# gsw4869/CUDA_LDPC

Measured on AMD Instinct MI355X. Metric: decoded codewords/sec (50-iter flooding min-sum, fixed iterations), higher is better.
Workload: dtype f32; 1 GPU; J4_L24_Z96 rate-0.833 batch=65536 codewords/GPU 50 iters Es/N0=3.0dB; kernel=qc_lds_halfrow-local<nf2,J4,L24,Z96,wc20,wv4,g4,w6>t768_lds79904, frames_per_gpu=65536

## Files before the change

__graft_entry__.py:

```python
import glob
import os
import subprocess
import sys

ROOT = os.path.dirname(os.path.abspath(__file__))
PKG = os.path.join(ROOT, "cuda_ldpc_amd")
CSRC = os.path.join(PKG, "csrc")
SO = os.path.join(PKG, "libcuda_ldpc_amd.so")
HIPCC = os.environ.get("HIPCC", "/opt/rocm/bin/hipcc")
HIP_FLAGS = ["-O3", "--offload-arch=gfx950", "-std=c++17", "-fPIC", "-shared", "-ffp-contract=off", "-Wall",
             "-Wno-unused-function"]


def _stale(target, sources):
    if not os.path.exists(target):
        return True
    t = os.path.getmtime(target)
    return any(os.path.getmtime(s) > t for s in sources)


def _unit_deps(unit):
    fam = os.path.basename(unit).split("_")[0]
    deps = [unit] + glob.glob(os.path.join(CSRC, "common*.hpp")) + glob.glob(os.path.join(ROOT, "include", "*.h"))
    with open(unit) as f:
        named = [line.split('"')[1] for line in f if line.startswith('#include "') and line.count('"') == 2]
    deps += [h for h in (os.path.join(CSRC, n) for n in named) if os.path.isfile(h)]
    for pat in ("*.hpp", "*.inc"):
        deps += [h for h in glob.glob(os.path.join(CSRC, pat)) if os.path.basename(h).startswith(fam + "_")]
    return deps


def build(force=False):
    units = sorted(glob.glob(os.path.join(CSRC, "*.hip")))
    objdir = os.path.join(ROOT, "build", "obj")
    os.makedirs(objdir, exist_ok=True)
    flags = [f for f in HIP_FLAGS if f != "-shared"]
    jobs, objs = [], []
    for u in units:
        o = os.path.join(objdir, os.path.basename(u)[:-4] + ".o")
        objs.append(o)
        if force or _stale(o, _unit_deps(u) + [os.path.abspath(__file__)]):
            cmd = [HIPCC] + flags + ["-I", os.path.join(ROOT, "include"), "-c", u, "-o", o]
            print("[build]", " ".join(cmd), flush=True)
            jobs.append((cmd, subprocess.Popen(cmd)))
    for cmd, p in jobs:
        if p.wait() != 0:
            raise subprocess.CalledProcessError(p.returncode, cmd)
    if force or jobs or _stale(SO, objs):
        cmd = [HIPCC, "--offload-arch=gfx950", "-shared", "-fPIC", "-o", SO] + objs
        print("[build]", " ".join(cmd), flush=True)
        subprocess.check_call(cmd)
    if ROOT not in sys.path:
        sys.path.insert(0, ROOT)
    from oracle import pyoracle
    pyoracle.build(force=force)
    import cuda_ldpc_amd
    return SO


def smoke():
    import numpy as np
    import torch
    if ROOT not in sys.path:
        sys.path.insert(0, ROOT)
    if not os.path.exists(SO):
        build()
    import cuda_ldpc_amd as C
    from oracle import pyoracle as orc
    assert torch.cuda.is_available(), "smoke() needs a GPU"
    torch.cuda.set_device(0)
    J, L, Z, F, iters = 4, 24, 96, 16, 10
    path = os.path.join(ROOT, "data", "bldpc", "J4_L24_Z96_BlockH.txt")
    seed = np.array([173, 173, 173], np.int32)
    y = orc.bldpc_awgn(seed, orc.bldpc_sigma(3.0), L * Z, F)
    want = orc.bldpc_decode(orc.BinaryCode(path, J, L, Z), y, F, iters, early_exit=0, want_app=True)
    code = C.BinaryCode.from_blockh(path, J, L, Z)
    yt = torch.from_numpy(y.reshape(L * Z, F)).cuda()
    for kern in (C.KERNEL_QC_LDS, C.KERNEL_TABLE):
        r = C.LDPC_Decoder_GPU(code, yt, max_iter=iters, exit_mode=C.EXIT_FIXED, kernel=kern, want_app=True)
        torch.cuda.synchronize()
        assert np.array_equal(r["D"].cpu().numpy().reshape(-1), want["D"]), "hard bits differ from the oracle"
        assert np.array_equal(r["app"].cpu().numpy().reshape(-1).view(np.uint32), want["app"].view(np.uint32)), "LLRs differ"
        print("[smoke] binary J4_L24_Z96 F=%d iters=%d kernel=%s: bit-exact vs oracle" % (F, iters, code.last_kernel))
    J, L, Z, F = 15, 30, 1280, 3
    path = os.path.join(ROOT, "data", "bldpc", "J15_L30_Z1280_BlockH.txt")
    seed = np.array([173, 173, 173], np.int32)
    y = orc.bldpc_awgn(seed, orc.bldpc_sigma(0.4), L * Z, F)
    want = orc.bldpc_decode(orc.BinaryCode(path, J, L, Z), y, F, 30, early_exit=1, want_app=True)
    code = C.BinaryCode.from_blockh(path, J, L, Z)
    r = C.LDPC_Decoder_GPU(code, torch.from_numpy(y.reshape(L * Z, F)).cuda(), max_iter=30, exit_mode=C.EXIT_BATCH_GLOBAL, want_app=True)
    torch.cuda.synchronize()
    assert r["iteraTime"] == want["it"] and np.array_equal(r["D"].cpu().numpy().reshape(-1), want["D"]), "J15_L30_Z1280 differs from the oracle"
    assert np.array_equal(r["app"].cpu().numpy().reshape(-1).view(np.uint32), want["app"].view(np.uint32)), "J15_L30_Z1280 LLRs differ"
    print("[smoke] binary J15_L30_Z1280 F=%d iteraTime=%d kernel=%s: bit-exact vs oracle" % (F, r["iteraTime"], code.last_kernel))
    from cuda_ldpc_amd import nbldpc as nb
    nbd = os.path.join(ROOT, "data", "nb")
    mul, _, _ = nb.GFInitial(64, os.path.join(nbd, "GF", "Arith.Table.GF.64.txt"))
    ncode = nb.NBCode(os.path.join(nbd, "BDS.576.288.GF.64.txt"), mul)
    ocode = orc.NBCode(os.path.join(nbd, "BDS.576.288.GF.64.txt"), os.path.join(nbd, "GF", "Arith.Table.GF.64.txt"))
    cw = np.loadtxt(os.path.join(nbd, "codeword_bds_gf64.txt"), dtype=np.int32)
    seed = np.array([173, 173, 173], np.int32)
    sigma = nb.sigma_of(3.0, ncode.rate)
    rx = np.stack([nb.AWGNChannel_CPU(seed, sigma, ncode, cw) for _ in range(4)])
    Lch = nb.Demodulate(ncode, torch.from_numpy(rx).cuda(), sigma)
    r = nb.Decoding_EMS(ncode, Lch, 2, 2, 20, want_state=True)
    torch.cuda.synchronize()
    for b in range(4):
        want = orc.nb_ems_decode(ocode, orc.nb_demodulate(ocode, rx[b], sigma), 2, 2, 20, want_state=True)
        assert np.array_equal(r["DecodeOutput"][b].cpu().numpy(), want["out"]), "NB symbols differ from the oracle"
        assert int(r["iter_number"][b]) == want["it"] and int(r["ok"][b]) == want["ok"]
        assert np.array_equal(r["LLR"][b].cpu().numpy().view(np.uint32), want["LLR"].view(np.uint32)), "NB LLRs differ"
    print("[smoke] NB BDS GF(64) N=96: 4 frames, iterations %s: bit-exact vs oracle" % r["iter_number"].cpu().tolist())
    r2 = nb.Decoding_EMS(ncode, Lch, 2, 2, 20, want_state="llr")
    torch.cuda.synchronize()
    for k in ("DecodeOutput", "iter_number", "ok"):
        assert torch.equal(r[k], r2[k]), "k_nb_ems2 differs from k_nb_ems: " + k
    assert torch.equal(r["LLR"].view(torch.int32), r2["LLR"].view(torch.int32)), "k_nb_ems2 LLRs differ"
    print("[smoke] NB BDS GF(64): two-frame pipeline kernel bit-exact as well")
    r4 = nb.Decoding_QSPA(ncode, Lch, 20, want_state=True)
    want = nb.Decoding_QSPA_host(ncode, Lch.cpu().numpy(), 20, want_state=True)
    torch.cuda.synchronize()
    for k in ("DecodeOutput", "iter_number", "ok"):
        assert np.array_equal(r4[k].cpu().numpy(), want[k]), "k_nb_qspa differs from the host statement: " + k
    for k in ("LLR", "L_c2v"):
        assert np.array_equal(r4[k].cpu().numpy().view(np.uint32), want[k].view(np.uint32)), "k_nb_qspa state differs: " + k
    print("[smoke] NB BDS GF(64): FHT sum-product, iterations %s: bit-exact vs host statement" % r4["iter_number"].cpu().tolist())
    r5 = nb.Decoding_QSPA(ncode, Lch, 20, want_state=True, layered=True)
    want = nb.Decoding_QSPA_host(ncode, Lch.cpu().numpy(), 20, want_state=True, layered=True)
    torch.cuda.synchronize()
    for k in ("DecodeOutput", "iter_number", "ok"):
        assert np.array_equal(r5[k].cpu().numpy(), want[k]), "k_nb_qspa_layered differs from the host statement: " + k
    for k in ("LLR", "L_c2v"):
        assert np.array_equal(r5[k].cpu().numpy().view(np.uint32), want[k].view(np.uint32)), "k_nb_qspa_layered state differs: " + k
    print("[smoke] NB BDS GF(64): layered FHT sum-product, iterations %s: bit-exact vs host statement" % r5["iter_number"].cpu().tolist())
    for layered, ref in ((False, r4), (True, r5)):
        rw = nb.Decoding_QSPA(ncode, Lch, 20, want_state=True, layered=layered, tier="workspace")
        torch.cuda.synchronize()
        assert ncode.last_kernel == ("k_nb_qspa_ws_layered" if layered else "k_nb_qspa_ws")
        for k in ("DecodeOutput", "iter_number", "ok", "LLR", "L_c2v"):
            assert torch.equal(rw[k].view(torch.int32), ref[k].view(torch.int32)), "%s differs from the LDS tier: %s" % (ncode.last_kernel, k)
    print("[smoke] NB BDS GF(64): FHT sum-product, workspace tier, both schedules: bit-exact vs the LDS tier")
    rm = C.RateMatch(ncode.N, [0, 5], range(88, 96))
    words = nb.PN_CodeWords(ncode, 1, 4, rate_match=rm)
    rxq = nb.AWGNChannel_RM_GPU(np.array([173, 173, 173], np.int32), 0.6, rm, 64, nb.RM_Select(rm, words))
    Lrm = nb.RM_Demodulate_Recover(rm, 64, rxq, 0.6)
    want = nb.RM_Demodulate_Recover_host(rm, 64, rxq.cpu().numpy(), 0.6)
    assert np.array_equal(Lrm.cpu().numpy().view(np.uint32), want.view(np.uint32)), "NB rate-matched L_ch differs from the host statement"
    r3 = nb.Decoding_EMS(ncode, Lrm, 2, 2, 20)
    torch.cuda.synchronize()
    assert int((r3["DecodeOutput"][:, [0, 5]] != 0).sum()) == 0, "a shortened symbol decoded to a non-zero element"
    print("[smoke] NB BDS GF(64) rate-matched (2 shortened, 8 punctured, E=%d): fused receive bit-exact vs host statement, %d of 4 frames ok"
          % (rm.E, int(r3["ok"].sum())))


if __name__ == "__main__":
    build(force="--force" in sys.argv)
    if "--smoke" in sys.argv:
        smoke()
```

cuda_ldpc_amd/csrc/bldpc_math.hpp:

```cpp
#pragma once
#include <hip/hip_runtime.h>
#include <stdint.h>
#define BLDPC_SELECT_FN __device__ __forceinline__
#include "bldpc_select.hpp"

namespace cldpc {

__device__ __forceinline__ uint32_t f2u(float x) { return __float_as_uint(x); }
__device__ __forceinline__ float u2f(uint32_t x) { return __uint_as_float(x); }

struct CnAcc {
    float m1, m2;
    uint32_t sgn;
    __device__ __forceinline__ void init()
    {
        m1 = __builtin_inff();
        m2 = __builtin_inff();
        sgn = 0u;
    }
    __device__ __forceinline__ void add(float q)
    {
        float a = __builtin_fabsf(q);
        sgn ^= f2u(q);
        m2 = __builtin_amdgcn_fmed3f(m1, m2, a);
        m1 = __builtin_fminf(m1, a);
    }
    __device__ __forceinline__ uint32_t key() const { return __builtin_amdgcn_bitop3_b32(f2u(m1), f2u(m2), sgn & 0x80000000u, 0x96); }
};

struct SelF32 {
    static __device__ __forceinline__ float min(float a, float b) { return __builtin_fminf(a, b); }
    static __device__ __forceinline__ float max(float a, float b) { return __builtin_fmaxf(a, b); }
    static __device__ __forceinline__ float min3(float a, float b, float c) { return __builtin_fminf(__builtin_fminf(a, b), c); }
    static __device__ __forceinline__ float med3(float a, float b, float c) { return __builtin_amdgcn_fmed3f(a, b, c); }
};

template <int N, int STRIDE> __device__ __forceinline__ void cn_two_smallest(const float *q, float &m1, float &m2, uint32_t &sgn)
{
    static_assert(N >= 2, "a check row half has at least two edges");
    float mag[N];
#pragma unroll
    for (int i = 0; i < N; i++) mag[i] = __builtin_fabsf(q[i * STRIDE]);
    two_smallest<SelF32, N, float>(mag, m1, m2);
#ifdef QC_XOR2
    sgn = 0u;
#pragma unroll
    for (int k = 0; k < N; k++) sgn ^= f2u(q[k * STRIDE]);
#else
    sgn = (N % 2) ? f2u(q[0]) : (f2u(q[0]) ^ f2u(q[STRIDE]));
#pragma unroll
    for (int k = 2 - (N % 2); k + 1 < N; k += 2) sgn = __builtin_amdgcn_bitop3_b32(sgn, f2u(q[k * STRIDE]), f2u(q[(k + 1) * STRIDE]), 0x96);
#endif
}

__device__ __forceinline__ float cn_out(float q, float m2, uint32_t key)
{
    return u2f(key ^ f2u(__builtin_amdgcn_fmed3f(q, -m2, m2)));
}

}
```

cuda_ldpc_amd/csrc/bldpc_qc2_body.inc:

```
template <typename GM, bool HIST, bool NORM = false> __global__ __launch_bounds__(GM::TPB, GM::MINW) void QC2_NAME(QcArgs a)
{
    constexpr int NF = GM::NF, L = GM::L, Z = GM::Z, WC = GM::WC, WV = GM::WV, GJ = GM::GJ, ZB = GM::ZB, WCH = GM::WCH;
    constexpr int RPT = GM::RPT, CPT = GM::CPT, NCG = GM::NCG, MSG = GM::MSG;
    static_assert(NF == 2, "the half-row kernel carries a frame pair per lane");
    constexpr bool LOC = GM::LOC;
    constexpr int NL = LOC ? CPT : 0;
    extern __shared__ __attribute__((aligned(16))) char lds[];
    const int chunk = (a.nWG + 7) >> 3;
#if QC2_PERSIST
    const int xcd = (int)(blockIdx.x & 7);
    int wg = 0;
#else
    const int wg = (int)(blockIdx.x & 7) * chunk + (int)(blockIdx.x >> 3);
    if (wg >= a.nWG) return;
#endif

    const int F = a.F;
    const int tid = threadIdx.x;
    const int wave = tid >> 6, lane = tid & 63, h = lane >> 5;
    const int jq = wave / ZB, t = (wave - jq * ZB) * 32 + (lane & 31);
    const int cg = jq * 2 + h;
#if QC2_PERSIST
    int f0 = 0;
#else
    const int f0 = wg * NF;
#endif
    int *lds_flag = reinterpret_cast<int *>(lds + GM::flag_byte);

    const int rbase = ((jq * WC + h * WCH) * Z + t) * MSG;
    const int sbase = (GM::Sslot + cg * Z + t) * MSG;
    int saddr[RPT][WCH];
    v2f32 Rr[RPT][WCH];
    int sst[LOC ? CPT : 1];
    int raddr[CPT][WV];
    {
        constexpr int NV = LOC ? CPT : 0, WVR = LOC ? WV - 1 : WV;
        int w[4 * GM::LW];
#pragma unroll
        for (int k = 0; k < GM::LW; k++) {
            const v4i32 x = a.lane[k * GM::TPB + tid];
            w[4 * k] = x.x; w[4 * k + 1] = x.y; w[4 * k + 2] = x.z; w[4 * k + 3] = x.w;
        }
#pragma unroll
        for (int cc = 0; cc < NV; cc++) sst[LOC ? cc : 0] = (GM::Sslot + w[cc]) * MSG;
#pragma unroll
        for (int rr = 0; rr < RPT; rr++)
#pragma unroll
            for (int i = 0; i < WCH; i++) saddr[rr][i] = w[NV + rr * WCH + i];
#pragma unroll
        for (int cc = 0; cc < CPT; cc++)
#pragma unroll
            for (int k = 0; k < WVR; k++) raddr[cc][k] = w[NV + RPT * WCH + cc * WVR + k];
    }
    v2f32 yreg[CPT];
    auto y_load = [&](int cc) -> v2f32 {
        const int n = LOC ? sst[LOC ? cc : 0] / MSG - GM::Sslot : (cg + cc * NCG) * Z + t;
        return a.y_raw ? *reinterpret_cast<const v2f32 *>(a.y_raw + (size_t)n * F + f0)
                       : *reinterpret_cast<const v2f32 *>(a.y + ((size_t)wg * (L * Z) + n) * NF);
    };
#if !QC2_PERSIST
#pragma unroll
    for (int cc = 0; cc < CPT; cc++) yreg[cc] = y_load(cc);
#endif
    if (tid < NF) {
        reinterpret_cast<float *>(lds)[GM::zero_slot * NF + tid] = 0.0f;
        reinterpret_cast<float *>(lds)[GM::inf_slot * NF + tid] = __builtin_inff();
        lds_flag[tid] = 0;
        lds_flag[NF + tid] = 0;
    }
    unsigned long long hist = 0;
    unsigned done = 0;
    constexpr unsigned ALL = (1u << NF) - 1u;
#ifdef QC_STAMPS
    int nst = 0;
    auto stamp = [&](unsigned long long v) { if (tid == 0 && nst < QC_STAMPS) a.stamps[(size_t)wg * QC_STAMPS + nst++] = v; };
    const unsigned hwid = __builtin_amdgcn_s_getreg((31 << 11) | 4), xcc = __builtin_amdgcn_s_getreg((31 << 11) | 20);
    stamp(((unsigned long long)xcc << 32) | hwid);
    stamp(__builtin_amdgcn_s_memtime());
    if (a.stagger && ((hwid >> 16) & 1))
        for (int i = 0; i < a.stagger; i += 64 * 16) __builtin_amdgcn_s_sleep(16);
#endif
#if !QC2_PERSIST
    __syncthreads();
#endif
#ifdef QC_STAMPS
    stamp(__builtin_amdgcn_s_memtime());
#endif

    auto vn_phase = [&](auto ZS, bool (&bad)[NF]) {
        constexpr bool zs = decltype(ZS)::value;
        constexpr int CB = (CPT * WV <= 12) ? CPT : 1;
        static_for<CPT / CB>([&](auto C0) {
            constexpr int c0 = decltype(C0)::value * CB;
            v2f32 R[CB][WV];
#pragma unroll
            for (int ci = 0; ci < CB; ci++)
#pragma unroll
                for (int k = 0; k < WV; k++) R[ci][k] = lds_ld2(raddr[c0 + ci][k]);
            static_for<CB>([&](auto CI) {
                constexpr int ci = decltype(CI)::value, cc = c0 + ci;
                v2f32 S = R[ci][0];
                if constexpr (zs) S = v2f32{0.0f, 0.0f} + S;
#pragma unroll
                for (int k = 1; k < WV; k++) S = S + R[ci][k];
                S = S + yreg[cc];
                lds_st2_imm<cc * NCG * Z * MSG>(sbase, S);
                if (HIST) {
                    const bool in_len = ((cg + cc * NCG) * Z + t) < a.length;
                    bad[0] = bad[0] || (in_len && S.x < 0);
                    bad[1] = bad[1] || (in_len && S.y < 0);
                }
            });
            if (CB < CPT) __builtin_amdgcn_sched_barrier(0);
        });
        asm volatile("s_waitcnt lgkmcnt(0)" ::: "memory");
    };
    v2f32 Sloc[LOC ? CPT : 1];
    const int jqs = __builtin_amdgcn_readfirstlane(jq);
    auto vn_phase_loc = [&](auto JJ, auto ZS, bool (&bad)[NF]) {
        constexpr int jj = decltype(JJ)::value;
        constexpr bool zs = decltype(ZS)::value;
        v2f32 R[CPT][WV - 1];
#pragma unroll
        for (int cc = 0; cc < CPT; cc++)
#pragma unroll
            for (int kk = 0; kk < WV - 1; kk++) R[cc][kk] = lds_ld2(raddr[cc][kk]);
        static_for<CPT>([&](auto CC) {
            constexpr int cc = decltype(CC)::value;
            v2f32 S = v2f32{0.0f, 0.0f};
            static_for<WV>([&](auto K) {
                constexpr int k = decltype(K)::value;
                v2f32 Rk;
                if constexpr (k == jj) Rk = Rr[0][cc];
                else Rk = R[cc][k - (k > jj ? 1 : 0)];
                if constexpr (k == 0 && !zs) S = Rk;
                else S = S + Rk;
            });
            S = S + yreg[cc];
            Sloc[LOC ? cc : 0] = S;
            lds_st2_imm<0>(sst[LOC ? cc : 0], S);
            if (HIST) {
                const bool in_len = (sst[LOC ? cc : 0] / MSG - GM::Sslot) < a.length;
                bad[0] = bad[0] || (in_len && S.x < 0);
                bad[1] = bad[1] || (in_len && S.y < 0);
            }
        });
        asm volatile("s_waitcnt lgkmcnt(0)" ::: "memory");
    };
    auto vn_first = [&](bool (&bad)[NF]) {
        static_for<CPT>([&](auto CC) {
            constexpr int cc = decltype(CC)::value;
            const v2f32 S = yreg[cc] + v2f32{0.0f, 0.0f};
            int n;
            if constexpr (LOC) {
                Sloc[LOC ? cc : 0] = S;
                lds_st2_imm<0>(sst[LOC ? cc : 0], S);
                n = sst[LOC ? cc : 0] / MSG - GM::Sslot;
            } else {
                lds_st2_imm<cc * NCG * Z * MSG>(sbase, S);
                n = (cg + cc * NCG) * Z + t;
            }
            if (HIST) {
                const bool in_len = n < a.length;
                bad[0] = bad[0] || (in_len && S.x < 0);
                bad[1] = bad[1] || (in_len && S.y < 0);
            }
        });
        asm volatile("s_waitcnt lgkmcnt(0)" ::: "memory");
    };
    auto vn_any = [&](bool (&bad)[NF]) {
        if constexpr (LOC) static_for<GM::J>([&](auto JJ) { if (jqs == decltype(JJ)::value) vn_phase_loc(JJ, std::true_type{}, bad); });
        else vn_phase(std::true_type{}, bad);
    };
    auto flags_publish = [&](const bool (&bad)[NF], int it) {
#pragma unroll
        for (int v = 0; v < NF; v++)
            if (bad[v]) lds_flag[(it & 1) * NF + v] = 1;
    };
    auto flags_collect = [&](int it) -> int {
        int flag = 0;
        if (tid < NF) {
            flag = lds_flag[(it & 1) * NF + tid] ? 0 : 1;
            lds_flag[((it + 1) & 1) * NF + tid] = 0;
            if (flag && it <= 64) hist |= (1ull << (it - 1));
        }
        return flag;
    };
    auto emit = [&](unsigned mask, bool (&bad)[NF]) {
        unsigned *obits = a.bits;
        float *oapp = a.app;
        asm volatile("" : "+s"(obits), "+s"(oapp));
#pragma unroll
        for (int cc = 0; cc < CPT; cc++) {
            const int n = (cg + cc * NCG) * Z + t;
            float S[NF];
            lds_ld<NF>(S, lds, sbase + cc * NCG * Z * MSG);
#pragma unroll
            for (int v = 0; v < NF; v++) {
                if (HIST && !((mask >> v) & 1u)) continue;
                const bool neg = S[v] < 0;
                if (!HIST) bad[v] = bad[v] || (n < a.length && neg);
                const unsigned long long m = __ballot(neg);
                if ((tid & 31) == 0 && f0 + v < F) obits[(size_t)(f0 + v) * GM::NW + (n >> 5)] = (unsigned)(m >> (tid & 32));
                if (oapp && f0 + v < F) oapp[(size_t)n * F + f0 + v] = S[v];
            }
        }
    };
    auto retire = [&](int it) -> bool {
        unsigned newly = 0;
#pragma unroll
        for (int v = 0; v < NF; v++)
            if (!lds_flag[(it & 1) * NF + v]) newly |= 1u << v;
        newly &= ~done;
        if (newly) {
            bool unused[NF];
            emit(newly, unused);
            if (tid < NF && ((newly >> tid) & 1u) && f0 + tid < F) a.iters[f0 + tid] = it;
            done |= newly;
        }
        return done == ALL;
    };

#if QC2_PERSIST
    for (;;) {
    if (tid == 0) lds_flag[0] = atomicAdd(&a.work[xcd], 1);
    __syncthreads();
    {
        const int ord = __builtin_amdgcn_readfirstlane(lds_flag[0]);
        if (ord >= chunk || xcd * chunk + ord >= a.nWG) break;
        wg = xcd * chunk + ord;
    }
    __syncthreads();
    f0 = wg * NF;
#pragma unroll
    for (int cc = 0; cc < CPT; cc++) yreg[cc] = y_load(cc);
    if (tid < NF) {
        lds_flag[tid] = 0;
        lds_flag[NF + tid] = 0;
    }
    hist = 0;
    done = 0;
    __syncthreads();
#endif
    auto iteration = [&](auto JJ, auto FIRST, int it) -> bool {
        constexpr bool first = decltype(FIRST)::value;
        bool bad[NF];
#pragma unroll
        for (int v = 0; v < NF; v++) bad[v] = false;
        __builtin_amdgcn_s_setprio(QC_PRIO_VN);
        if constexpr (first) vn_first(bad);
        else if constexpr (LOC) vn_phase_loc(JJ, std::bool_constant<HIST>{}, bad);
        else vn_phase(std::bool_constant<HIST>{}, bad);
        if (HIST) flags_publish(bad, it);
        __syncthreads();
        __builtin_amdgcn_s_setprio(QC_PRIO_CN);
#ifdef QC_STAMPS
        stamp(__builtin_amdgcn_s_memtime());
#endif
        if (HIST) {
            (void)flags_collect(it);
            if (a.per_frame && retire(it)) return true;
        }

#pragma unroll
        for (int rr = 0; rr < RPT; rr++) {
            CnAcc acc[NF];
            {
#ifdef QC2_CHK_SPLIT
                constexpr int CHK = (WCH > 6) ? (WCH + 1) / 2 : WCH;
#else
                constexpr int CHK = (WCH > 6 && !LOC) ? (WCH + 1) / 2 : WCH;
#endif
#pragma unroll
                for (int c0 = 0; c0 < WCH; c0 += CHK) {
                    v2f32 Sv[CHK];
#pragma unroll
                    for (int i = 0; i < CHK && c0 + i < WCH; i++) {
                        if (LOC && c0 + i < NL) Sv[i] = Sloc[LOC ? c0 + i : 0];
                        else Sv[i] = lds_ld2(saddr[rr][c0 + i]);
                    }
#pragma unroll
                    for (int i = 0; i < CHK && c0 + i < WCH; i++) Rr[rr][c0 + i] = first ? Sv[i] : Sv[i] - Rr[rr][c0 + i];
                    if (c0 + CHK < WCH) __builtin_amdgcn_sched_barrier(0);
                }
            }
#if QC_ACC_RUNNING
#pragma unroll
            for (int v = 0; v < NF; v++) acc[v].init();
#pragma unroll
            for (int i = 0; i < WCH; i++) {
                acc[0].add(Rr[rr][i].x);
                acc[1].add(Rr[rr][i].y);
            }
#else
            cn_two_smallest<WCH, 2>(reinterpret_cast<const float *>(&Rr[rr][0]), acc[0].m1, acc[0].m2, acc[0].sgn);
            cn_two_smallest<WCH, 2>(reinterpret_cast<const float *>(&Rr[rr][0]) + 1, acc[1].m1, acc[1].m2, acc[1].sgn);
#endif
            uint32_t a1 = f2u(acc[0].m1), b1 = f2u(acc[1].m1), a2 = f2u(acc[0].m2), b2 = f2u(acc[1].m2), as = acc[0].sgn, bs = acc[1].sgn;
            swap32(a1, b1);
            swap32(a2, b2);
            swap32(as, bs);
            const uint32_t m1 = min(a1, b1);
            uint32_t m2u = min(min(max(a1, b1), a2), b2);
            uint32_t keyu = __builtin_amdgcn_bitop3_b32(m1, m2u, __builtin_amdgcn_bitop3_b32(as, bs, 0x80000000u, 0x28), 0x96);
            uint32_t m2v = m2u, keyv = keyu;
            swap32(m2u, m2v);
            swap32(keyu, keyv);
            const float m2f[NF] = {u2f(m2u), u2f(m2v)};
            const uint32_t key[NF] = {keyu, keyv};
            __builtin_amdgcn_s_setprio(LOC ? QC_PRIO_WR_LOC : QC_PRIO_WR);
            static_for<RPT * WCH>([&](auto I) {
                constexpr int r_ = decltype(I)::value / WCH, i = decltype(I)::value % WCH;
                if (r_ != rr) return;
                v2f32 Rn;
                Rn.x = cn_out(Rr[rr][i].x, m2f[0], key[0]);
                Rn.y = cn_out(Rr[rr][i].y, m2f[1], key[1]);
                if constexpr (NORM) Rn = Rn * a.alpha;
                Rr[rr][i] = Rn;
                if constexpr (!(LOC && i < NL)) lds_st2_imm<(r_ * GJ * WC + i) * Z * MSG>(rbase, Rn);
            });
        }
        asm volatile("s_waitcnt lgkmcnt(0)" ::: "memory");
        __syncthreads();
#ifdef QC_STAMPS
        stamp(__builtin_amdgcn_s_memtime());
#endif
        return false;
    };
    const bool retired = a.max_iter > 1 && iteration(std::integral_constant<int, 0>{}, std::true_type{}, 1);
    auto iterate = [&](auto JJ) {
        for (int it = 2; it < a.max_iter; it++)
            if (iteration(JJ, std::false_type{}, it)) return;
    };
    if (!retired) {
        if constexpr (LOC) static_for<GM::J>([&](auto JJ) { if (jqs == decltype(JJ)::value) iterate(JJ); });
        else iterate(std::integral_constant<int, 0>{});
    }

    int flag = 0;
    if (!(HIST && done == ALL)) {
        bool bad[NF];
#pragma unroll
        for (int v = 0; v < NF; v++) bad[v] = false;
        if (a.max_iter > 1) vn_any(bad);
        else vn_first(bad);
        if (LOC) __syncthreads();
        emit(~done, bad);
        flags_publish(bad, a.max_iter);
        __syncthreads();
        flag = flags_collect(a.max_iter);
    }
#ifdef QC_STAMPS
    stamp(__builtin_amdgcn_s_memtime());
#endif
    if (tid < NF && f0 + tid < F) {
        const bool stopped = HIST && ((done >> tid) & 1u);
        a.D[(size_t)L * Z * F + f0 + tid] = stopped ? 1 : flag;
        if (HIST && a.hist) a.hist[f0 + tid] = hist;
        if (HIST && a.per_frame && !stopped) a.iters[f0 + tid] = a.max_iter;
    }
#if QC2_PERSIST
    __syncthreads();
    }
#endif
}
```

cuda_ldpc_amd/csrc/bldpc_select.hpp:

```cpp
#pragma once

#ifndef BLDPC_SELECT_FN
#define BLDPC_SELECT_FN inline
#endif

namespace cldpc {

template <typename P, int N, typename T> BLDPC_SELECT_FN void two_smallest(const T (&v)[N], T &m1, T &m2)
{
    static_assert(N >= 2, "two values at least");
    if constexpr (N == 2) {
        m1 = P::min(v[0], v[1]);
        m2 = P::max(v[0], v[1]);
    } else if constexpr (N == 3) {
        m1 = P::min3(v[0], v[1], v[2]);
        m2 = P::med3(v[0], v[1], v[2]);
    } else if constexpr (N == 4) {
        const T lo = P::min3(v[0], v[1], v[2]), mid = P::med3(v[0], v[1], v[2]);
        m2 = P::med3(lo, mid, v[3]);
        m1 = P::min(lo, v[3]);
    } else {
        constexpr int K = N / 3, R = N % 3;
        T low[K + R], mid[K];
#pragma unroll
        for (int k = 0; k < K; k++) {
            low[k] = P::min3(v[3 * k], v[3 * k + 1], v[3 * k + 2]);
            mid[k] = P::med3(v[3 * k], v[3 * k + 1], v[3 * k + 2]);
        }
#pragma unroll
        for (int r = 0; r < R; r++) low[K + r] = v[3 * K + r];
        two_smallest<P, K + R, T>(low, m1, m2);
#pragma unroll
        for (int k = 0; k + 2 <= K; k += 2) m2 = P::min3(m2, mid[k], mid[k + 1]);
        if constexpr (K % 2) m2 = P::min(m2, mid[K - 1]);
    }
}

}
```

Baseline: 14.41 million codewords/s.

## Pre-compute local-edge check partials during the VN phase LDS wait

Before the final LDS wait of the variable-node phase, the kernel now computes the check-node min/med/sign partials for the first three register-resident (local) edges. The check-node phase then only folds in the remaining edges, using an abs-folding selector that puts the fabs into instruction modifiers. The write-back loop is rotated so local edges come last. The aim is to hide ALU work behind outstanding LDS latency and to shorten the check-node critical path, at the cost of extra live registers across the phase boundary. Test-program builds are also added to the build script.

```diff
diff --git a/__graft_entry__.py b/__graft_entry__.py
--- a/__graft_entry__.py
+++ b/__graft_entry__.py
@@ -30,6 +30,22 @@
     return deps
 
 
+TEST_PROGRAMS = [("qc2_local_width_%d" % w, "qc2_local_width_test.hip", ["-DHALF_ROW=%d" % w]) for w in (8, 9)]
+TEST_BIN = os.path.join(ROOT, "build", "tests")
+
+
+def stale_test_programs(force=False):
+    os.makedirs(TEST_BIN, exist_ok=True)
+    jobs = []
+    for name, src, defs in TEST_PROGRAMS:
+        exe, src = os.path.join(TEST_BIN, name), os.path.join(ROOT, "tests", "cpp", src)
+        deps = [src, os.path.abspath(__file__)] + _unit_deps(os.path.join(CSRC, "bldpc_api.hip"))[1:]
+        if force or _stale(exe, deps):
+            jobs.append(([HIPCC, "-O3", "--offload-arch=gfx950", "-std=c++17", "-ffp-contract=off", "-Wno-unused-function"] + defs
+                         + ["-I", os.path.join(ROOT, "include"), src, "-o", exe], exe))
+    return jobs
+
+
 def build(force=False):
     units = sorted(glob.glob(os.path.join(CSRC, "*.hip")))
     objdir = os.path.join(ROOT, "build", "obj")
@@ -43,10 +59,14 @@
             cmd = [HIPCC] + flags + ["-I", os.path.join(ROOT, "include"), "-c", u, "-o", o]
             print("[build]", " ".join(cmd), flush=True)
             jobs.append((cmd, subprocess.Popen(cmd)))
+    n_units = len(jobs)
+    for cmd, _ in stale_test_programs(force):
+        print("[build]", " ".join(cmd), flush=True)
+        jobs.append((cmd, subprocess.Popen(cmd)))
     for cmd, p in jobs:
         if p.wait() != 0:
             raise subprocess.CalledProcessError(p.returncode, cmd)
-    if force or jobs or _stale(SO, objs):
+    if force or n_units or _stale(SO, objs):
         cmd = [HIPCC, "--offload-arch=gfx950", "-shared", "-fPIC", "-o", SO] + objs
         print("[build]", " ".join(cmd), flush=True)
         subprocess.check_call(cmd)
diff --git a/cuda_ldpc_amd/csrc/bldpc_math.hpp b/cuda_ldpc_amd/csrc/bldpc_math.hpp
--- a/cuda_ldpc_amd/csrc/bldpc_math.hpp
+++ b/cuda_ldpc_amd/csrc/bldpc_math.hpp
@@ -35,6 +35,18 @@
     static __device__ __forceinline__ float med3(float a, float b, float c) { return __builtin_amdgcn_fmed3f(a, b, c); }
 };
 
+struct SelAbsF32 {
+    static __device__ __forceinline__ float min(float a, float b)
+    {
+        float r;
+        asm("v_min_f32_e64 %0, |%1|, |%2|" : "=v"(r) : "v"(a), "v"(b));
+        return r;
+    }
+    static __device__ __forceinline__ float max(float a, float b) { return __builtin_fmaxf(__builtin_fabsf(a), __builtin_fabsf(b)); }
+    static __device__ __forceinline__ float min3(float a, float b, float c) { return __builtin_fminf(__builtin_fminf(__builtin_fabsf(a), __builtin_fabsf(b)), __builtin_fabsf(c)); }
+    static __device__ __forceinline__ float med3(float a, float b, float c) { return __builtin_amdgcn_fmed3f(__builtin_fabsf(a), __builtin_fabsf(b), __builtin_fabsf(c)); }
+};
+
 template <int N, int STRIDE> __device__ __forceinline__ void cn_two_smallest(const float *q, float &m1, float &m2, uint32_t &sgn)
 {
     static_assert(N >= 2, "a check row half has at least two edges");
@@ -53,6 +65,26 @@
 #endif
 }
 
+template <int STRIDE> __device__ __forceinline__ void cn_lead_triple(const float *q, float &lo, float &mid, uint32_t &sgn)
+{
+    const float a = __builtin_fabsf(q[0]), b = __builtin_fabsf(q[STRIDE]), c = __builtin_fabsf(q[2 * STRIDE]);
+    lo = SelF32::min3(a, b, c);
+    mid = SelF32::med3(a, b, c);
+    sgn = __builtin_amdgcn_bitop3_b32(f2u(q[0]), f2u(q[STRIDE]), f2u(q[2 * STRIDE]), 0x96);
+}
+template <int N, int STRIDE> __device__ __forceinline__ void cn_two_smallest_lead(float lo, float mid, uint32_t sgn3, const float *q, float &m1, float &m2, uint32_t &sgn)
+{
+    static_assert(N >= 4, "the first triple and one edge more at least");
+    float raw[N - 3];
+#pragma unroll
+    for (int i = 0; i < N - 3; i++) raw[i] = q[i * STRIDE];
+    two_smallest_lead<SelAbsF32, N, float>(lo, mid, raw, m1, m2);
+    sgn = sgn3;
+#pragma unroll
+    for (int k = 0; k + 1 < N - 3; k += 2) sgn = __builtin_amdgcn_bitop3_b32(sgn, f2u(q[k * STRIDE]), f2u(q[(k + 1) * STRIDE]), 0x96);
+    if constexpr ((N - 3) % 2) sgn ^= f2u(q[(N - 4) * STRIDE]);
+}
+
 __device__ __forceinline__ float cn_out(float q, float m2, uint32_t key)
 {
     return u2f(key ^ f2u(__builtin_amdgcn_fmed3f(q, -m2, m2)));
diff --git a/cuda_ldpc_amd/csrc/bldpc_qc2_body.inc b/cuda_ldpc_amd/csrc/bldpc_qc2_body.inc
--- a/cuda_ldpc_amd/csrc/bldpc_qc2_body.inc
+++ b/cuda_ldpc_amd/csrc/bldpc_qc2_body.inc
@@ -117,7 +117,7 @@
     };
     v2f32 Sloc[LOC ? CPT : 1];
     const int jqs = __builtin_amdgcn_readfirstlane(jq);
-    auto vn_phase_loc = [&](auto JJ, auto ZS, bool (&bad)[NF]) {
+    auto vn_phase_loc = [&](auto JJ, auto ZS, bool (&bad)[NF], auto &&pre_wait) {
         constexpr int jj = decltype(JJ)::value;
         constexpr bool zs = decltype(ZS)::value;
         v2f32 R[CPT][WV - 1];
@@ -145,9 +145,10 @@
                 bad[1] = bad[1] || (in_len && S.y < 0);
             }
         });
+        pre_wait();
         asm volatile("s_waitcnt lgkmcnt(0)" ::: "memory");
     };
-    auto vn_first = [&](bool (&bad)[NF]) {
+    auto vn_first = [&](bool (&bad)[NF], auto &&pre_wait) {
         static_for<CPT>([&](auto CC) {
             constexpr int cc = decltype(CC)::value;
             const v2f32 S = yreg[cc] + v2f32{0.0f, 0.0f};
@@ -166,10 +167,12 @@
                 bad[1] = bad[1] || (in_len && S.y < 0);
             }
         });
+        pre_wait();
         asm volatile("s_waitcnt lgkmcnt(0)" ::: "memory");
     };
+    auto no_early = []() {};
     auto vn_any = [&](bool (&bad)[NF]) {
-        if constexpr (LOC) static_for<GM::J>([&](auto JJ) { if (jqs == decltype(JJ)::value) vn_phase_loc(JJ, std::true_type{}, bad); });
+        if constexpr (LOC) static_for<GM::J>([&](auto JJ) { if (jqs == decltype(JJ)::value) vn_phase_loc(JJ, std::true_type{}, bad, no_early); });
         else vn_phase(std::true_type{}, bad);
     };
     auto flags_publish = [&](const bool (&bad)[NF], int it) {
@@ -242,14 +245,30 @@
     done = 0;
     __syncthreads();
 #endif
+    constexpr int NE = (NL >= 3 && WCH >= 4) ? 3 : 0;
+    float elo[NF], emid[NF];
+    uint32_t esg[NF];
+    auto cn_local = [&](auto FIRST) {
+        constexpr bool first = decltype(FIRST)::value;
+#pragma unroll
+        for (int i = 0; i < NL; i++) Rr[0][i] = first ? Sloc[LOC ? i : 0] : Sloc[LOC ? i : 0] - Rr[0][i];
+#pragma unroll
+        for (int v = 0; v < NF; v++) cn_lead_triple<2>(reinterpret_cast<const float *>(&Rr[0][0]) + v, elo[v], emid[v], esg[v]);
+    };
     auto iteration = [&](auto JJ, auto FIRST, int it) -> bool {
         constexpr bool first = decltype(FIRST)::value;
         bool bad[NF];
 #pragma unroll
         for (int v = 0; v < NF; v++) bad[v] = false;
         __builtin_amdgcn_s_setprio(QC_PRIO_VN);
-        if constexpr (first) vn_first(bad);
-        else if constexpr (LOC) vn_phase_loc(JJ, std::bool_constant<HIST>{}, bad);
+        auto early = [&]() {
+            if constexpr (NE > 0) {
+                cn_local(FIRST);
+                __builtin_amdgcn_sched_barrier(0);
+            }
+        };
+        if constexpr (first) vn_first(bad, early);
+        else if constexpr (LOC) vn_phase_loc(JJ, std::bool_constant<HIST>{}, bad, early);
         else vn_phase(std::bool_constant<HIST>{}, bad);
         if (HIST) flags_publish(bad, it);
         __syncthreads();
@@ -280,11 +299,13 @@
                         else Sv[i] = lds_ld2(saddr[rr][c0 + i]);
                     }
 #pragma unroll
-                    for (int i = 0; i < CHK && c0 + i < WCH; i++) Rr[rr][c0 + i] = first ? Sv[i] : Sv[i] - Rr[rr][c0 + i];
+                    for (int i = 0; i < CHK && c0 + i < WCH; i++)
+                        if (!(NE > 0 && c0 + i < NL)) Rr[rr][c0 + i] = first ? Sv[i] : Sv[i] - Rr[rr][c0 + i];
                     if (c0 + CHK < WCH) __builtin_amdgcn_sched_barrier(0);
                 }
             }
 #if QC_ACC_RUNNING
+            static_assert(NE == 0, "the running accumulator takes every edge");
 #pragma unroll
             for (int v = 0; v < NF; v++) acc[v].init();
 #pragma unroll
@@ -293,8 +314,14 @@
                 acc[1].add(Rr[rr][i].y);
             }
 #else
-            cn_two_smallest<WCH, 2>(reinterpret_cast<const float *>(&Rr[rr][0]), acc[0].m1, acc[0].m2, acc[0].sgn);
-            cn_two_smallest<WCH, 2>(reinterpret_cast<const float *>(&Rr[rr][0]) + 1, acc[1].m1, acc[1].m2, acc[1].sgn);
+            if constexpr (NE > 0) {
+#pragma unroll
+                for (int v = 0; v < NF; v++)
+                    cn_two_smallest_lead<WCH, 2>(elo[v], emid[v], esg[v], reinterpret_cast<const float *>(&Rr[rr][NE]) + v, acc[v].m1, acc[v].m2, acc[v].sgn);
+            } else {
+                cn_two_smallest<WCH, 2>(reinterpret_cast<const float *>(&Rr[rr][0]), acc[0].m1, acc[0].m2, acc[0].sgn);
+                cn_two_smallest<WCH, 2>(reinterpret_cast<const float *>(&Rr[rr][0]) + 1, acc[1].m1, acc[1].m2, acc[1].sgn);
+            }
 #endif
             uint32_t a1 = f2u(acc[0].m1), b1 = f2u(acc[1].m1), a2 = f2u(acc[0].m2), b2 = f2u(acc[1].m2), as = acc[0].sgn, bs = acc[1].sgn;
             swap32(a1, b1);
@@ -310,7 +337,7 @@
             const uint32_t key[NF] = {keyu, keyv};
             __builtin_amdgcn_s_setprio(LOC ? QC_PRIO_WR_LOC : QC_PRIO_WR);
             static_for<RPT * WCH>([&](auto I) {
-                constexpr int r_ = decltype(I)::value / WCH, i = decltype(I)::value % WCH;
+                constexpr int r_ = decltype(I)::value / WCH, i = (decltype(I)::value % WCH + NL) % WCH;
                 if (r_ != rr) return;
                 v2f32 Rn;
                 Rn.x = cn_out(Rr[rr][i].x, m2f[0], key[0]);
@@ -320,6 +347,7 @@
                 if constexpr (!(LOC && i < NL)) lds_st2_imm<(r_ * GJ * WC + i) * Z * MSG>(rbase, Rn);
             });
         }
+        if (NL > 0) __builtin_amdgcn_sched_barrier(0);
         asm volatile("s_waitcnt lgkmcnt(0)" ::: "memory");
         __syncthreads();
 #ifdef QC_STAMPS
@@ -343,7 +371,7 @@
 #pragma unroll
         for (int v = 0; v < NF; v++) bad[v] = false;
         if (a.max_iter > 1) vn_any(bad);
-        else vn_first(bad);
+        else vn_first(bad, no_early);
         if (LOC) __syncthreads();
         emit(~done, bad);
         flags_publish(bad, a.max_iter);
diff --git a/cuda_ldpc_amd/csrc/bldpc_select.hpp b/cuda_ldpc_amd/csrc/bldpc_select.hpp
--- a/cuda_ldpc_amd/csrc/bldpc_select.hpp
+++ b/cuda_ldpc_amd/csrc/bldpc_select.hpp
@@ -36,4 +36,29 @@
     }
 }
 
+template <typename P, int N, typename T> BLDPC_SELECT_FN void two_smallest_lead(T lo0, T mid0, const T (&rest)[N - 3], T &m1, T &m2)
+{
+    static_assert(N >= 4, "the first triple and one value more at least");
+    if constexpr (N == 4) {
+        m2 = P::med3(lo0, mid0, rest[0]);
+        m1 = P::min(lo0, rest[0]);
+    } else {
+        constexpr int K = N / 3, R = N % 3;
+        T low[K + R], mid[K];
+        low[0] = lo0;
+        mid[0] = mid0;
+#pragma unroll
+        for (int k = 1; k < K; k++) {
+            low[k] = P::min3(rest[3 * k - 3], rest[3 * k - 2], rest[3 * k - 1]);
+            mid[k] = P::med3(rest[3 * k - 3], rest[3 * k - 2], rest[3 * k - 1]);
+        }
+#pragma unroll
+        for (int r = 0; r < R; r++) low[K + r] = rest[3 * K - 3 + r];
+        two_smallest<P, K + R, T>(low, m1, m2);
+#pragma unroll
+        for (int k = 0; k + 2 <= K; k += 2) m2 = P::min3(m2, mid[k], mid[k + 1]);
+        if constexpr (K % 2) m2 = P::min(m2, mid[K - 1]);
+    }
 }
+
+}
```

Measured after the change: 15.23 million codewords/s (median of 6 runs). 1.06x the previous value.
